# ukeSJTU/tiaozhanbei-unet

Hardware: AMD Instinct MI355X
Metric: training images/sec, AnomalyUNet 256x256 bs=32 per GPU (higher is better)
Workload: dtype bf16; 1 GPU; AnomalyUNet 3x256x256, bs=32/GPU, MSE+focal loss, Adam (BASELINE.json configs[2], synthetic randn images, bernoulli masks); global_batch=32, parallelism=dp1, accumulate=fp32, master_params=fp32, dist_world=1, reserved_cus=0, cu_budget=256

## Files before the change

tiaozhanbei_unet_amd/csrc/elementwise.hip:

```cpp
#include "common.h"

namespace {

inline int ew_blocks(long long items) { return (int)std::min<long long>(cdiv64(items, 256), 256 * 16); }

template <typename T>
__global__ __launch_bounds__(256) void nchw_to_nhwc_kernel(const float* __restrict__ src, T* __restrict__ dst,
                                                           int N, int C, int H, int W, int Cp) {
  constexpr int PIECE = ET<T>::PIECE;
  const long long hw = (long long)H * W;
  const long long total = (long long)N * hw;
  for (long long i = blockIdx.x * (long long)blockDim.x + threadIdx.x; i < total;
       i += (long long)gridDim.x * blockDim.x) {
    const long long n = i / hw, p = i - n * hw;
    const float* s = src + n * C * hw + p;
    T* o = dst + i * Cp;
    for (int c0 = 0; c0 < Cp; c0 += PIECE) {
      float v[PIECE];
#pragma unroll
      for (int j = 0; j < PIECE; ++j) v[j] = (c0 + j < C) ? s[(long long)(c0 + j) * hw] : 0.f;
      Vec<T>::store(o + c0, v);
    }
  }
}

template <typename T>
__global__ void nhwc_to_nchw_kernel(const T* __restrict__ src, float* __restrict__ dst, int N, int C, int H,
                                    int W, int Cp) {
  const long long hw = (long long)H * W;
  const long long total = (long long)N * C * hw;
  for (long long i = blockIdx.x * (long long)blockDim.x + threadIdx.x; i < total;
       i += (long long)gridDim.x * blockDim.x) {
    const long long p = i % hw;
    const long long t = i / hw;
    const int c = (int)(t % C);
    const long long n = t / C;
    dst[i] = ET<T>::to_f(src[(n * hw + p) * Cp + c]);
  }
}

template <typename T>
__global__ void pack_weight_kernel(const float* __restrict__ w, T* __restrict__ out, int Co, int Ci, int rows,
                                   int K, int mode, long long total, const float* __restrict__ scale) {
  for (long long i = blockIdx.x * (long long)blockDim.x + threadIdx.x; i < total;
       i += (long long)gridDim.x * blockDim.x) {
    float v = 0.f;
    if (mode == UNET_PACK_CONV_FWD) {
      const int ci = (int)(i % K);
      long long t = i / K;
      const int co = (int)(t % rows);
      const int tap = (int)(t / rows);
      if (co < Co && ci < Ci) v = w[((long long)co * Ci + ci) * 9 + tap] * (scale ? scale[co] : 1.f);
    } else if (mode == UNET_PACK_CONV_DGRAD) {
      const int co = (int)(i % K);
      long long t = i / K;
      const int ci = (int)(t % rows);
      const int tap = (int)(t / rows);
      if (co < Co && ci < Ci) v = w[((long long)co * Ci + ci) * 9 + (8 - tap)];
    } else if (mode == UNET_PACK_CONVT_FWD) {
      const int ci = (int)(i % K);
      long long t = i / K;
      const int co = (int)(t % rows);
      const int z = (int)(t / rows);
      if (co < Co && ci < Ci) v = w[((long long)ci * Co + co) * 4 + z];
    } else {
      const int co = (int)(i % K);
      long long t = i / K;
      const int z = (int)(t % 4);
      const int ci = (int)(t / 4);
      if (co < Co && ci < Ci) v = w[((long long)ci * Co + co) * 4 + z];
    }
    out[i] = ET<T>::from_f(v);
  }
}

template <typename T>
__global__ __launch_bounds__(256) void pack_weights_batched_kernel(const unet_pack_desc* __restrict__ descs) {
  __shared__ float tile[32 * 289];
  const unet_pack_desc d = descs[blockIdx.y];
  const int mode = d.mode;
  if (d.reserved > 0 && mode <= UNET_PACK_CONV_DGRAD) {
    const long long total = 9LL * d.rows * d.k;
    T* __restrict__ out = reinterpret_cast<T*>(d.out);
    for (long long i = blockIdx.x * 256LL + threadIdx.x; i < total; i += (long long)gridDim.x * 256)
      out[i] = ET<T>::from_f(unet_pack_seg_value(d.w, d.c_out, d.c_in, d.rows, d.k, mode, d.reserved, i, nullptr));
    return;
  }
  if constexpr (sizeof(T) == 2) {
    auto pair_ok = [](const unet_pack_desc& f, const unet_pack_desc& g) {
      return f.mode == UNET_PACK_CONV_FWD && g.mode == UNET_PACK_CONV_DGRAD && f.w == g.w && f.c_out == g.c_out &&
             f.c_in == g.c_in && f.rows == f.c_out && f.k == f.c_in && g.rows == g.c_in && g.k == g.c_out &&
             (f.c_out & 31) == 0 && (f.c_in & 31) == 0;
    };
    if (mode == UNET_PACK_CONV_DGRAD && blockIdx.y > 0 && pair_ok(descs[blockIdx.y - 1], d)) return;
    if (mode == UNET_PACK_CONV_FWD && blockIdx.y + 1 < gridDim.y && pair_ok(d, descs[blockIdx.y + 1])) {
      const unet_pack_desc g = descs[blockIdx.y + 1];
      const int Co = d.c_out, Ci = d.c_in;
      const int nB = Ci / 32, ntile = (Co / 32) * nB;
      const float* __restrict__ w = d.w;
      bf16_t* __restrict__ of = reinterpret_cast<bf16_t*>(d.out);
      bf16_t* __restrict__ og = reinterpret_cast<bf16_t*>(g.out);
      for (int t = blockIdx.x; t < ntile; t += gridDim.x) {
        const int a0 = (t / nB) * 32, b0 = (t % nB) * 32;
        __syncthreads();
        for (int i = threadIdx.x; i < 32 * 288; i += 256) {
          const int al = i / 288, r = i - al * 288;
          tile[al * 289 + r] = w[((size_t)(a0 + al) * Ci + b0) * 9 + r];
        }
        __syncthreads();
        for (int gi = threadIdx.x; gi < 2 * 32 * 9 * 4; gi += 256) {
          const int lay = gi / (32 * 9 * 4), rem = gi % (32 * 9 * 4);
          const int q = rem & 3, rest = rem >> 2;
          const int tap = rest % 9, outer = rest / 9;
          bf16x8 r8;
          if (lay == 0) {
#pragma unroll
            for (int e = 0; e < 8; ++e) r8[e] = (bf16_t)tile[outer * 289 + (q * 8 + e) * 9 + tap];
            *reinterpret_cast<bf16x8*>(of + ((size_t)tap * Co + a0 + outer) * Ci + b0 + q * 8) = r8;
          } else {
#pragma unroll
            for (int e = 0; e < 8; ++e) r8[e] = (bf16_t)tile[(q * 8 + e) * 289 + outer * 9 + tap];
            *reinterpret_cast<bf16x8*>(og + ((size_t)(8 - tap) * Ci + b0 + outer) * Co + a0 + q * 8) = r8;
          }
        }
      }
      return;
    }
  }
  const bool conv = mode <= UNET_PACK_CONV_DGRAD;
  const int taps = conv ? 9 : 4;
  const int As = conv ? d.c_out : d.c_in, Bs = conv ? d.c_in : d.c_out;
  const bool along_b = (mode == UNET_PACK_CONV_FWD || mode == UNET_PACK_CONVT_DGRAD);
  const int Ap = (mode == UNET_PACK_CONV_FWD || mode == UNET_PACK_CONVT_DGRAD) ? d.rows : d.k;
  const int Bp = (mode == UNET_PACK_CONV_FWD || mode == UNET_PACK_CONVT_DGRAD) ? d.k : d.rows;
  const int TA = along_b ? 8 : 64, TB = along_b ? 64 : 8;
  const int nA = (Ap + TA - 1) / TA, nB = (Bp + TB - 1) / TB;
  const float* __restrict__ w = d.w;
  T* __restrict__ out = reinterpret_cast<T*>(d.out);
  const int run = TB * taps;
  for (int t = blockIdx.x; t < nA * nB; t += gridDim.x) {
    const int a0 = (t / nB) * TA, b0 = (t % nB) * TB;
    __syncthreads();
    for (int i = threadIdx.x; i < TA * run; i += 256) {
      const int al = i / run, r = i - al * run;
      const int a = a0 + al, bb = b0 + r / taps;
      tile[i] = (a < As && bb < Bs) ? w[((size_t)a * Bs + b0) * taps + r] : 0.f;
    }
    __syncthreads();
    if ((((along_b ? Bp : Ap) & 7) == 0) && ((d.k & 7) == 0)) {
      for (int gi = threadIdx.x; gi < TA * TB * taps / 8; gi += 256) {
        const int inner0 = (gi & 7) * 8, rest = gi >> 3;
        const int tap = rest % taps, outer = rest / taps;
        const int al0 = along_b ? outer : inner0, bl0 = along_b ? inner0 : outer;
        const int a = a0 + al0, bb = b0 + bl0;
        if (a >= Ap || bb >= Bp) continue;
        float v[8];
#pragma unroll
        for (int e = 0; e < 8; ++e) v[e] = tile[(al0 + (along_b ? 0 : e)) * run + (bl0 + (along_b ? e : 0)) * taps + tap];
        size_t o;
        if (mode == UNET_PACK_CONV_FWD) o = ((size_t)tap * d.rows + a) * d.k + bb;
        else if (mode == UNET_PACK_CONV_DGRAD) o = ((size_t)(8 - tap) * d.rows + bb) * d.k + a;
        else if (mode == UNET_PACK_CONVT_FWD) o = ((size_t)tap * d.rows + bb) * d.k + a;
        else o = ((size_t)a * 4 + tap) * d.k + bb;
        if constexpr (sizeof(T) == 2) {
          bf16x8 r;
#pragma unroll
          for (int e = 0; e < 8; ++e) r[e] = (bf16_t)v[e];
          *reinterpret_cast<bf16x8*>(out + o) = r;
        } else {
          *reinterpret_cast<f32x4*>(out + o) = f32x4{v[0], v[1], v[2], v[3]};
          *reinterpret_cast<f32x4*>(out + o + 4) = f32x4{v[4], v[5], v[6], v[7]};
        }
      }
      continue;
    }
    for (int i = threadIdx.x; i < TA * TB * taps; i += 256) {
      const int inner = i & 63, rest = i >> 6;
      const int tap = rest % taps, outer = rest / taps;
      const int al = along_b ? outer : inner, bl = along_b ? inner : outer;
      const int a = a0 + al, bb = b0 + bl;
      if (a >= Ap || bb >= Bp) continue;
      const float v = tile[al * run + bl * taps + tap];
      size_t o;
      if (mode == UNET_PACK_CONV_FWD) o = ((size_t)tap * d.rows + a) * d.k + bb;
      else if (mode == UNET_PACK_CONV_DGRAD) o = ((size_t)(8 - tap) * d.rows + bb) * d.k + a;
      else if (mode == UNET_PACK_CONVT_FWD) o = ((size_t)tap * d.rows + bb) * d.k + a;
      else o = ((size_t)a * 4 + tap) * d.k + bb;
      out[o] = ET<T>::from_f(v);
    }
  }
}

template <typename T>
__global__ void maxpool2_fwd_kernel(const T* __restrict__ x, T* __restrict__ y, int N, int H, int W, int C) {
  constexpr int PIECE = ET<T>::PIECE;
  const int OH = H / 2, OW = W / 2, G = C / PIECE;
  const long long total = (long long)N * OH * OW * G;
  for (long long i = blockIdx.x * (long long)blockDim.x + threadIdx.x; i < total;
       i += (long long)gridDim.x * blockDim.x) {
    const int g = (int)(i % G);
    long long t = i / G;
    const int ox = (int)(t % OW);  t /= OW;
    const int oy = (int)(t % OH);
    const long long n = t / OH;
    const T* p = x + ((n * H + 2 * oy) * W + 2 * ox) * (long long)C + g * PIECE;
    float a[PIECE], b[PIECE], c[PIECE], d[PIECE];
    Vec<T>::load(p, a);
    Vec<T>::load(p + C, b);
    Vec<T>::load(p + (long long)W * C, c);
    Vec<T>::load(p + (long long)W * C + C, d);
#pragma unroll
    for (int j = 0; j < PIECE; ++j) a[j] = fmaxf(fmaxf(a[j], b[j]), fmaxf(c[j], d[j]));
    Vec<T>::store(y + i * PIECE, a);
  }
}

template <typename T>
__global__ void maxpool2_bwd_kernel(const T* __restrict__ x, const T* __restrict__ dy, T* __restrict__ dx,
                                    int N, int H, int W, int C, int accumulate) {
  constexpr int PIECE = ET<T>::PIECE;
  const int OH = H / 2, OW = W / 2, G = C / PIECE;
  const int WH = (H + 1) / 2, WW = (W + 1) / 2;
  const long long total = (long long)N * WH * WW * G;
  for (long long i = blockIdx.x * (long long)blockDim.x + threadIdx.x; i < total;
       i += (long long)gridDim.x * blockDim.x) {
    const int g = (int)(i % G);
    long long t = i / G;
    const int ox = (int)(t % WW);  t /= WW;
    const int oy = (int)(t % WH);
    const long long n = t / WH;
    const long long base = ((n * H + 2 * oy) * W + 2 * ox) * (long long)C + g * PIECE;
    float z[PIECE];
#pragma unroll
    for (int j = 0; j < PIECE; ++j) z[j] = 0.f;
    if (oy < OH && ox < OW) {
      float a[PIECE], b[PIECE], c[PIECE], d[PIECE], gr[PIECE];
      Vec<T>::load(x + base, a);
      Vec<T>::load(x + base + C, b);
      Vec<T>::load(x + base + (long long)W * C, c);
      Vec<T>::load(x + base + (long long)W * C + C, d);
      Vec<T>::load(dy + (((n * OH + oy) * OW + ox) * (long long)C + g * PIECE), gr);
      float ga[PIECE], gb[PIECE], gc[PIECE], gd[PIECE];
// ... 347 lines not shown
    using T = decltype(tag);
    return ew_launch("nchw_to_nhwc_kernel", nchw_to_nhwc_kernel<T>, (long long)n * h * w, UNET_K_PACK, stream, src, (T*)dst,
                     n, c, h, w, c_pad);
  });
}

extern "C" int32_t unet_nhwc_to_nchw(const void* src, float* dst, int32_t n, int32_t c, int32_t h, int32_t w,
                                     int32_t c_pad, int32_t dtype, void* stream) {
  UNET_REQUIRE(src && dst, UNET_ERR_BAD_ARG, "unet_nhwc_to_nchw: null pointer");
  UNET_REQUIRE(n > 0 && c > 0 && h > 0 && w > 0 && c_pad >= c, UNET_ERR_BAD_ARG, "unet_nhwc_to_nchw: bad dims");
  return with_dtype("unet_nhwc_to_nchw", dtype, [&](auto tag) {
    using T = decltype(tag);
    return ew_launch("nhwc_to_nchw_kernel", nhwc_to_nchw_kernel<T>, (long long)n * h * w * c, UNET_K_PACK, stream,
                     (const T*)src, dst, n, c, h, w, c_pad);
  });
}

static int32_t launch_pack_weight(const char* who, int dtype, const float* w, void* out, int c_out, int c_in, int rows, int k,
                                  int mode, int taps, const float* scale, void* stream) {
  const long long total = (long long)taps * rows * k;
  return with_dtype(who, dtype, [&](auto tag) {
    using T = decltype(tag);
    return ew_launch("pack_weight_kernel", pack_weight_kernel<T>, total, UNET_K_PACK, stream, w, (T*)out, c_out, c_in, rows,
                     k, mode, total, scale);
  });
}

extern "C" int32_t unet_pack_weight(const float* w, void* out, int32_t c_out, int32_t c_in, int32_t rows,
                                    int32_t k, int32_t mode, int32_t dtype, void* stream) {
  UNET_REQUIRE(w && out, UNET_ERR_BAD_ARG, "unet_pack_weight: null pointer");
  UNET_REQUIRE(c_out > 0 && c_in > 0 && rows > 0 && k > 0 && mode >= 0 && mode <= 3, UNET_ERR_BAD_ARG,
               "unet_pack_weight: bad dims/mode");
  const int gemm_rows = (mode == UNET_PACK_CONV_FWD || mode == UNET_PACK_CONVT_FWD) ? c_out : c_in;
  const int gemm_k = (mode == UNET_PACK_CONV_FWD || mode == UNET_PACK_CONVT_FWD) ? c_in : c_out;
  UNET_REQUIRE(rows >= gemm_rows && k >= gemm_k, UNET_ERR_BAD_ARG, "unet_pack_weight: padded dims too small");
  const int taps = (mode <= UNET_PACK_CONV_DGRAD) ? 9 : 4;
  return launch_pack_weight("unet_pack_weight", dtype, w, out, c_out, c_in, rows, k, mode, taps, nullptr, stream);
}

extern "C" int32_t unet_pack_conv_weight_folded(const float* w, const float* scale, void* out, int32_t c_out, int32_t c_in,
                                                int32_t rows, int32_t k, int32_t dtype, void* stream) {
  UNET_REQUIRE(w && scale && out, UNET_ERR_BAD_ARG, "unet_pack_conv_weight_folded: null pointer");
  UNET_REQUIRE(c_out > 0 && c_in > 0 && rows >= c_out && k >= c_in, UNET_ERR_BAD_ARG, "unet_pack_conv_weight_folded: bad dims");
  return launch_pack_weight("unet_pack_conv_weight_folded", dtype, w, out, c_out, c_in, rows, k, UNET_PACK_CONV_FWD, 9, scale,
                            stream);
}

extern "C" int32_t unet_pack_weights_batched(const unet_pack_desc* descs, int32_t n, int32_t dtype, void* stream) {
  UNET_REQUIRE(descs && n > 0 && n <= 65535, UNET_ERR_BAD_ARG, "unet_pack_weights_batched: bad argument");
  hipStream_t s = (hipStream_t)stream;
  return with_dtype("unet_pack_weights_batched", dtype, [&](auto tag) {
    using T = decltype(tag);
    ProfScope prof(UNET_K_PACK, 0.0, s);
    hipLaunchKernelGGL(pack_weights_batched_kernel<T>, dim3(224, n), dim3(256), 0, s, descs);
    return unet_check_launch("pack_weights_batched_kernel");
  });
}

extern "C" int32_t unet_maxpool2_fwd(int32_t dtype, const void* x, int32_t n, int32_t h, int32_t w, int32_t c,
                                     void* y, void* stream) {
  UNET_REQUIRE(x && y, UNET_ERR_BAD_ARG, "unet_maxpool2_fwd: null pointer");
  UNET_REQUIRE(n > 0 && h >= 2 && w >= 2 && c > 0 && c % 8 == 0, UNET_ERR_UNSUPPORTED, "unet_maxpool2_fwd: dims");
  return with_dtype("unet_maxpool2_fwd", dtype, [&](auto tag) {
    using T = decltype(tag);
    const long long total = (long long)n * (h / 2) * (w / 2) * c / ET<T>::PIECE;
    return ew_launch("maxpool2_fwd_kernel", maxpool2_fwd_kernel<T>, total, UNET_K_POOL, stream, (const T*)x, (T*)y, n, h, w, c);
  });
}

extern "C" int32_t unet_maxpool2_bwd(int32_t dtype, const void* x, const void* dy, int32_t n, int32_t h,
                                     int32_t w, int32_t c, void* dx, int32_t accumulate, void* stream) {
  UNET_REQUIRE(x && dy && dx, UNET_ERR_BAD_ARG, "unet_maxpool2_bwd: null pointer");
  UNET_REQUIRE(n > 0 && h >= 2 && w >= 2 && c > 0 && c % 8 == 0, UNET_ERR_UNSUPPORTED, "unet_maxpool2_bwd: dims");
  return with_dtype("unet_maxpool2_bwd", dtype, [&](auto tag) {
    using T = decltype(tag);
    const long long total = (long long)n * ((h + 1) / 2) * ((w + 1) / 2) * c / ET<T>::PIECE;
    return ew_launch("maxpool2_bwd_kernel", maxpool2_bwd_kernel<T>, total, UNET_K_POOL, stream, (const T*)x, (const T*)dy,
                     (T*)dx, n, h, w, c, accumulate);
  });
}

extern "C" int32_t unet_bn_relu_pool_supported(int32_t dtype, int32_t c) {
  if (!dtype_known(dtype)) return 0;
  const int piece = dtype == UNET_BF16 ? ET<bf16_t>::PIECE : ET<float>::PIECE;
  return (c > 0 && c % piece == 0 && 256 % (c / piece) == 0) ? 1 : 0;
}

template <typename T> using PoolIdx32 = std::conditional_t<sizeof(T) == 2, int, long long>;

extern "C" int32_t unet_bn_relu_pool_fwd(int32_t dtype, const void* y, int32_t n, int32_t h, int32_t w, int32_t c,
                                         const float* scale, const float* shift, void* a, void* pooled, void* stream) {
  UNET_REQUIRE(y && scale && shift && a && pooled, UNET_ERR_BAD_ARG, "unet_bn_relu_pool_fwd: null pointer");
  hipStream_t s = (hipStream_t)stream;
  return with_dtype("unet_bn_relu_pool_fwd", dtype, [&](auto tag) -> int32_t {
    using T = decltype(tag);
    UNET_REQUIRE(n > 0 && h >= 2 && w >= 2 && unet_bn_relu_pool_supported(dtype, c), UNET_ERR_UNSUPPORTED,
                 "unet_bn_relu_pool_fwd: c=%d h=%d w=%d", c, h, w);
    ProfScope prof(UNET_K_BN, 0.0, s, "bn_relu_pool_fwd_kernel");
    const long long total = (long long)n * ((h + 1) / 2) * ((w + 1) / 2) * (c / ET<T>::PIECE);
    const dim3 grid(ew_blocks(total));
    if ((long long)n * h * w * c < 0x7FFFFFFFLL)
      hipLaunchKernelGGL((bn_relu_pool_fwd_kernel<T, PoolIdx32<T>>), grid, dim3(256), 0, s, (const T*)y, scale, shift, (T*)a,
                         (T*)pooled, n, h, w, c);
    else
      hipLaunchKernelGGL((bn_relu_pool_fwd_kernel<T, long long>), grid, dim3(256), 0, s, (const T*)y, scale, shift, (T*)a,
                         (T*)pooled, n, h, w, c);
    return unet_check_launch("bn_relu_pool_fwd_kernel");
// ... 274 lines not shown
```

tiaozhanbei_unet_amd/csrc/first.hip:

```cpp
#include <stdlib.h>

#include <algorithm>

#include "conv_common.h"

namespace {

constexpr unsigned OOB = 0xFFFFFFF0u;
constexpr int FIRST_CO = 64;

struct SegPos { int seg, y, n; };
__device__ __forceinline__ SegPos seg_step(SegPos p, int dseg, int dy, int dn, int segs_row, int H) {
  p.seg += dseg;
  int c = p.seg >= segs_row;
  p.seg -= c ? segs_row : 0;
  p.y += dy + c;
  c = p.y >= H;
  p.y -= c ? H : 0;
  p.n += dn + c;
  return p;
}
struct SegWalk { SegPos first; int dseg, dy, dn; };
__device__ __forceinline__ SegWalk seg_walk(long long u0, long long stride, int segs_row, int H) {
  SegWalk w;
  const long long r0 = u0 / segs_row, rs = stride / segs_row;
  w.first = SegPos{(int)(u0 - r0 * segs_row), (int)(r0 % H), (int)std::min<long long>(r0 / H, 1 << 30)};
  w.dseg = (int)(stride - rs * segs_row);
  w.dy = (int)(rs % H);
  w.dn = (int)std::min<long long>(rs / H, 1 << 28);
  return w;
}

struct FirstParams {
  const float* x;
  const float* w;
  char* y;
  float* part;
  int N, CI, H, W;
  const char* y_raw;
  const float* coefs;
};

__global__ __launch_bounds__(256, 3) void first_fwd_kernel(const FirstParams P) {
  __shared__ float red[4][2][FIRST_CO];
  const int tid = threadIdx.x, lane = tid & 63, wave = tid >> 6;
  const int l15 = lane & 15, kb = lane >> 4;
  const int K = 9 * P.CI;
  const int HW = P.H * P.W;

  bf16x8 wa[4];
#pragma unroll
  for (int ct = 0; ct < 4; ++ct)
#pragma unroll
    for (int e = 0; e < 8; ++e) {
      const int k = kb * 8 + e;
      float v = 0.f;
      if (k < K) {
// ... 247 lines not shown
  for (int i = 0; i < WU; ++i) issue_or_skip(seg_step(cur, i, 0, 0, segs_row, P.H), i, xc[i]);
  while (cur.n < P.N) {
    const SegPos nxt = seg_step(cur, wk.dseg, wk.dy, wk.dn, segs_row, P.H);
#pragma unroll
    for (int i = 0; i < WU; ++i) issue_or_skip(seg_step(nxt, i, 0, 0, segs_row, P.H), (buf ^ 1) * WU + i, xn[i]);
    asm volatile("s_waitcnt vmcnt(%0)" ::"n"(NV * WU) : "memory");
#pragma unroll
    for (int i = 0; i < WU; ++i) {
      bf16x8 fb;
#pragma unroll
      for (int e = 0; e < 8; ++e) fb[e] = (bf16_t)xc[i][e];
      const char* sb = wbuf + (buf * WU + i) * SEGB;
#pragma unroll
      for (int wr = 0; wr < 2; ++wr) {
        bf16x8 fa = tr_frag2(sb, aoff[wr], aoff[wr] + 4 * 128);
        if constexpr (BNB) {
          const bf16x8 fy = tr_frag2(sb + 2048, aoff[wr], aoff[wr] + 4 * 128);
#pragma unroll
          for (int e = 0; e < 8; ++e)
            fa[e] = (bf16_t)fmaf(cA[wr], (float)fa[e], fmaf(cB[wr], (float)fy[e], cK[wr]));
        }
        acc[wr] = __builtin_amdgcn_mfma_f32_32x32x16_bf16(fa, fb, acc[wr], 0, 0, 0);
      }
    }
#pragma unroll
    for (int i = 0; i < WU; ++i)
#pragma unroll
      for (int e = 0; e < 8; ++e) xc[i][e] = xn[i][e];
    buf ^= 1;
    cur = nxt;
  }
  asm volatile("s_waitcnt vmcnt(0)" ::: "memory");

  __syncthreads();
  float* red = reinterpret_cast<float*>(smem);
#pragma unroll
  for (int wr = 0; wr < 2; ++wr)
#pragma unroll
    for (int r = 0; r < 16; ++r) {
      const int co = wr * 32 + (r & 3) + 8 * (r >> 2) + 4 * hh;
      red[(wave * FIRST_CO + co) * 32 + l31] = acc[wr][r];
    }
  __syncthreads();
  for (int i = tid; i < FIRST_CO * 32; i += 256) {
    const float t = ((red[i] + red[FIRST_CO * 32 + i]) + red[2 * FIRST_CO * 32 + i]) + red[3 * FIRST_CO * 32 + i];
    P.part[(size_t)blockIdx.x * (FIRST_CO * 32) + i] = t;
  }
}

__global__ __launch_bounds__(256) void first_wgrad_reduce_kernel(const float* __restrict__ part, int nparts, int CI,
                                                                 float* __restrict__ dw) {
  __shared__ float red[8][32];
  const int co = blockIdx.x, k = threadIdx.x & 31, pl = threadIdx.x >> 5;
  float s0 = 0.f, s1 = 0.f;
  int b = pl;
  for (; b + 8 < nparts; b += 16) {
    s0 += part[(size_t)b * (FIRST_CO * 32) + co * 32 + k];
    s1 += part[(size_t)(b + 8) * (FIRST_CO * 32) + co * 32 + k];
  }
  if (b < nparts) s0 += part[(size_t)b * (FIRST_CO * 32) + co * 32 + k];
  red[pl][k] = s0 + s1;
  __syncthreads();
  if (threadIdx.x < 9 * CI) {
    const int kk = threadIdx.x, tap = kk / CI, ci = kk - tap * CI;
    float t = red[0][kk];
#pragma unroll
    for (int i = 1; i < 8; ++i) t += red[i][kk];
    dw[(co * CI + ci) * 9 + tap] = t;
  }
}

int first_blocks(long long units, int per_iter, int per_cu) {
  long long b = (units + 4 * per_iter - 1) / (4 * per_iter);
  return (int)std::min<long long>(b, 256 * per_cu);
}

}

extern "C" int32_t unet_conv3x3_first_supported(int32_t c_in, int32_t c_out, int32_t h, int32_t w) {
  return (c_in >= 1 && 9 * c_in <= 32 && c_out == FIRST_CO && h > 0 && w > 0 && w % 16 == 0) ? 1 : 0;
}

extern "C" int32_t unet_conv3x3_first_stats(int32_t n, int32_t h, int32_t w, const float* x, int32_t c_in,
                                            const float* weight, void* y, float* partial, int32_t* n_parts,
                                            void* stream) {
  UNET_REQUIRE(x && weight && y, UNET_ERR_BAD_ARG, "unet_conv3x3_first_stats: null pointer");
  UNET_REQUIRE(n > 0 && unet_conv3x3_first_supported(c_in, FIRST_CO, h, w), UNET_ERR_UNSUPPORTED,
               "unet_conv3x3_first_stats: n=%d c_in=%d h=%d w=%d (needs 9*c_in <= 32, w %% 16 == 0)", n, c_in, h, w);
  UNET_REQUIRE((long long)c_in * h * w * 4 < 0x7FFFFFFFLL, UNET_ERR_UNSUPPORTED, "unet_conv3x3_first_stats: image too large");
  const long long units = (long long)n * h * (w / 16);
  const int blocks = first_blocks(units, 2, 3);
  FirstParams P{x, weight, (char*)y, partial, n, c_in, h, w, nullptr, nullptr};
  hipStream_t s = (hipStream_t)stream;
  ProfScope prof(UNET_K_CONV_FWD, 2.0 * n * h * w * (double)FIRST_CO * c_in * 9, s);
  hipLaunchKernelGGL(first_fwd_kernel, dim3(blocks), dim3(256), 0, s, P);
  if (n_parts) *n_parts = partial ? blocks : 0;
  return unet_check_launch("first_fwd_kernel");
}

extern "C" size_t unet_conv3x3_first_wgrad_workspace(int32_t n, int32_t h, int32_t w) {
  const long long units = (long long)n * h * (w / 16 > 0 ? w / 16 : 1);
  return (size_t)first_blocks(units, 2, 4) * FIRST_CO * 32 * sizeof(float);
}

static int32_t first_wgrad_impl(int32_t n, int32_t h, int32_t w, const float* x, int32_t c_in, const void* dy, const void* y_raw,
                                const float* coefs, float* dw, void* workspace, size_t workspace_bytes, void* stream,
                                const char* what) {
  UNET_REQUIRE(x && dy && dw && workspace, UNET_ERR_BAD_ARG, "%s: null pointer", what);
  UNET_REQUIRE(n > 0 && unet_conv3x3_first_supported(c_in, FIRST_CO, h, w), UNET_ERR_UNSUPPORTED,
               "%s: n=%d c_in=%d h=%d w=%d", what, n, c_in, h, w);
  UNET_REQUIRE((long long)c_in * h * w * 4 < 0x7FFFFFFFLL, UNET_ERR_UNSUPPORTED, "%s: image too large", what);
  UNET_REQUIRE(workspace_bytes >= unet_conv3x3_first_wgrad_workspace(n, h, w), UNET_ERR_WORKSPACE, "%s: workspace too small", what);
  const long long units = (long long)n * h * (w / 16);
  const int blocks = first_blocks(units, 2, 4);
// ... 26 lines not shown
```

tiaozhanbei_unet_amd/csrc/wgrad.hip:

```cpp
#include <stdlib.h>

#include <algorithm>

#include "common.h"

namespace {

struct WView { const char* p; int C, H, W, oy, ox; };

#ifdef PDMA_STAMPS
void* g_wgrad_debug = nullptr;
#endif
struct WgradParams {
  void* debug;
  WView rt;
  WView ct[2];
  int N, H, W;
  int Crow, Ccol;
  float* partial;
  int split, tilesPerSplit, tilesX, tilesY, nR, nC;
  int xcd_chunk;
};

__device__ inline bool wgrad_block_coords(const WgradParams& P, int& sp, int& rtile, int& ctile) {
// ... 629 lines not shown
#pragma unroll
  for (int tap = 0; tap < 9; ++tap) {
    float* o = P.partial + ((size_t)(sp * 9 + tap) * P.Crow) * P.Ccol;
#pragma unroll
    for (int cb = 0; cb < 2; ++cb)
#pragma unroll
      for (int nb = 0; nb < 2; ++nb) {
        const int row = rch + wr * 32 + cb * 16 + i16;
        const int col = ctile * 64 + wc * 32 + nb * 16 + g * 4;
        *reinterpret_cast<f32x4*>(o + (size_t)row * P.Ccol + col) = acc[tap][cb][nb];
      }
  }
  asm volatile("s_waitcnt vmcnt(0)" ::: "memory");
#ifdef PDMA_STAMPS
  if (P.debug && lane == 0 && blockIdx.x < 256) {
    unsigned long long* o = (unsigned long long*)P.debug + ((size_t)blockIdx.x * 8 + wave) * 8;
    for (int i = 0; i < 4; ++i) o[i] = wg_st[i];
    o[4] = (unsigned long long)(t_end - t_begin);
    o[5] = ((__builtin_amdgcn_s_memtime() - wg_t0) << 20) / (__builtin_amdgcn_s_memrealtime() - wg_r0 + 1);
    o[6] = __builtin_amdgcn_s_memtime() - wg_e0;
    o[7] = __builtin_amdgcn_s_memtime() - wg_t0;
  }
#endif
}

template <int TAPS>
__global__ __launch_bounds__(256) void wgrad_reduce_wide_kernel(const float* __restrict__ partial,
                                                                float* __restrict__ out, int split, int Crow,
                                                                int Ccol, int rows_out, int cols_out) {
  __shared__ float red[4][64];
  const int cl = threadIdx.x & 63, ks = threadIdx.x >> 6;
  int b = blockIdx.x;
  const int tap = b % TAPS;  b /= TAPS;
  const int nchunk = (cols_out + 63) / 64;
  const int c = (b % nchunk) * 64 + cl, r = b / nchunk;
  const size_t plane = (size_t)Crow * Ccol, slab = (size_t)TAPS * plane;
  float s = 0.f;
  if (c < cols_out) {
    const float* p = partial + (size_t)tap * plane + (size_t)r * Ccol + c;
    int k = ks;
    for (; k + 12 < split; k += 16) {
      const float a0 = p[(size_t)k * slab], a1 = p[(size_t)(k + 4) * slab], a2 = p[(size_t)(k + 8) * slab],
                  a3 = p[(size_t)(k + 12) * slab];
      s += a0; s += a1; s += a2; s += a3;
    }
    for (; k < split; k += 4) s += p[(size_t)k * slab];
  }
  red[ks][cl] = s;
  __syncthreads();
  if (ks == 0 && c < cols_out)
    out[((size_t)r * cols_out + c) * TAPS + tap] = (red[0][cl] + red[1][cl]) + (red[2][cl] + red[3][cl]);
}

struct Plan { int tilesX, tilesY, nR, nC, split, tilesPerSplit; size_t bytes; };

template <int TAPS>
Plan make_plan(int n, int h, int w, int crow, int ccol) {
  Plan p;
  constexpr int TH = (TAPS == 9) ? 8 : 4;
  p.tilesX = cdiv(w, 16);
  p.tilesY = cdiv(h, TH);
  p.nR = crow / 64;
  p.nC = ccol / 64;
  const long long ntiles = (long long)n * p.tilesY * p.tilesX;
  long long want = 2LL * unet_cu_budget() / ((long long)p.nR * p.nC);
  if (want < 1) want = 1;
  if (want > ntiles) want = ntiles;
  p.tilesPerSplit = (int)cdiv64(ntiles, want);
  p.split = (int)cdiv64(ntiles, p.tilesPerSplit);
  p.bytes = (size_t)p.split * TAPS * crow * ccol * sizeof(float);
  return p;
}

inline Plan make_plan16(int n, int h, int w, int crow, int ccol) {
  Plan p;
  const bool paired = w <= 16;
  p.tilesX = paired ? 1 : cdiv(w, 32);
  p.tilesY = cdiv(h, 4);
  p.nR = crow / 128;
  p.nC = ccol / 64;
  const long long ntiles = (long long)(paired ? (n + 1) / 2 : n) * p.tilesY * p.tilesX;
  long long want = (long long)unet_cu_budget() / ((long long)p.nR * p.nC);
  if (want < 1) want = 1;
  if (want > ntiles) want = ntiles;
  p.tilesPerSplit = (int)cdiv64(ntiles, want);
  p.split = (int)cdiv64(ntiles, p.tilesPerSplit);
  p.bytes = (size_t)p.split * 9 * crow * ccol * sizeof(float);
  return p;
}

template <bool PAIRED>
void launch16(const WgradParams& P, long long blocks, hipStream_t s) {
  using C = W16<PAIRED>;
  auto kern = wgrad16_kernel<PAIRED>;
  unet_set_max_lds(reinterpret_cast<const void*>(kern), C::LDS);
  hipLaunchKernelGGL(kern, dim3((unsigned)blocks), dim3(512), C::LDS, s, P);
}

template <typename T, int TAPS>
int32_t run(WgradParams& P, const Plan& pl, float* out, int rows_out, int cols_out, int kclass, hipStream_t s) {
  P.tilesX = pl.tilesX; P.tilesY = pl.tilesY; P.nR = pl.nR; P.nC = pl.nC;
  P.split = pl.split; P.tilesPerSplit = pl.tilesPerSplit;
  long long blocks = (long long)pl.split * pl.nR * pl.nC;
  P.xcd_chunk = 0;
  if (blocks >= 16) {
    P.xcd_chunk = (int)cdiv64(blocks, 8);
    blocks = 8LL * P.xcd_chunk;
  }
  const double flops = 2.0 * P.N * P.H * P.W * (double)P.Crow * P.Ccol * TAPS;
  int split_used = pl.split;
  {
    const double alg_bytes = (double)P.N * P.H * P.W * ((double)P.Crow + P.Ccol * (TAPS == 9 ? 1.0 : 4.0)) * sizeof(T) +
                             4.0 * TAPS * rows_out * cols_out;
    constexpr bool DMA = sizeof(T) == 2 && TAPS == 9;
    const bool v16 = DMA && P.Crow % 128 == 0;
    ProfScope prof(kclass, flops, s,
                   v16 ? "wgrad16_kernel (+ reduce)" : (DMA ? "wgrad_dma_kernel (+ reduce)" : "wgrad_kernel (+ reduce)"), alg_bytes);
    if constexpr (DMA) {
      if (v16) {
        const Plan p16 = make_plan16(P.N, P.H, P.W, P.Crow, P.Ccol);
        P.tilesX = p16.tilesX; P.tilesY = p16.tilesY; P.nR = p16.nR; P.nC = p16.nC;
        P.split = p16.split; P.tilesPerSplit = p16.tilesPerSplit;
        split_used = p16.split;
        long long b16 = (long long)p16.split * p16.nR * p16.nC;
        P.xcd_chunk = 0;
        if (b16 >= 16) { P.xcd_chunk = (int)cdiv64(b16, 8); b16 = 8LL * P.xcd_chunk; }
        if (P.W <= 16) launch16<true>(P, b16, s);
        else launch16<false>(P, b16, s);
      } else {
        unet_set_max_lds(reinterpret_cast<const void*>(wgrad_dma_kernel), WDma::LDS);
        hipLaunchKernelGGL(wgrad_dma_kernel, dim3((unsigned)blocks), dim3(256), WDma::LDS, s, P);
      }
    } else {
      using C = WCfg<T, TAPS>;
      auto kern = wgrad_kernel<T, TAPS>;
      unet_set_max_lds(reinterpret_cast<const void*>(kern), C::LDS);
      hipLaunchKernelGGL(kern, dim3((unsigned)blocks), dim3(256), C::LDS, s, P);
    }
    int32_t rc = unet_check_launch("wgrad_kernel");
    if (rc) return rc;
    if (split_used >= 16) {
      const long long rb = (long long)rows_out * ((cols_out + 63) / 64) * TAPS;
      hipLaunchKernelGGL(wgrad_reduce_wide_kernel<TAPS>, dim3((unsigned)rb), dim3(256), 0, s, (const float*)P.partial,
                         out, split_used, P.Crow, P.Ccol, rows_out, cols_out);
    } else {
      const long long total = (long long)rows_out * cols_out;
      const int rb = (int)std::min<long long>(cdiv64(total, 256), 4096);
      hipLaunchKernelGGL(wgrad_reduce_kernel<TAPS>, dim3(rb), dim3(256), 0, s, (const float*)P.partial, out, split_used,
                         P.Crow, P.Ccol, rows_out, cols_out);
    }
  }
  return unet_check_launch("wgrad_reduce_kernel");
}

inline int pad64(int c) { return (c + 63) / 64 * 64; }

}

extern "C" size_t unet_conv3x3_wgrad_workspace(int32_t n, int32_t h, int32_t w, int32_t c_in, int32_t c_out) {
  size_t bytes = make_plan<9>(n, h, w, pad64(c_out), pad64(c_in)).bytes;
  if (pad64(c_out) % 128 == 0)
    bytes = std::max(bytes, make_plan16(n, h, w, pad64(c_out), pad64(c_in)).bytes);
  return bytes;
}

extern "C" int32_t unet_conv3x3_wgrad(int32_t dtype, int32_t n, int32_t h, int32_t w, const unet_view src[2],
                                      const void* dy, int32_t c_out, float* dw, int32_t c_in_param,
                                      void* workspace, size_t workspace_bytes, void* stream) {
  UNET_REQUIRE(src && src[0].ptr && dy && dw && workspace, UNET_ERR_BAD_ARG, "unet_conv3x3_wgrad: null pointer");
  UNET_REQUIRE(n > 0 && h > 0 && w > 0, UNET_ERR_BAD_ARG, "unet_conv3x3_wgrad: bad dims");
  const int ctot = src[0].c + (src[1].ptr ? src[1].c : 0);
  UNET_REQUIRE(c_out % 64 == 0, UNET_ERR_UNSUPPORTED, "unet_conv3x3_wgrad: c_out %d not a multiple of 64", c_out);
  UNET_REQUIRE(ctot % 64 == 0 && (!src[1].ptr || src[0].c % 64 == 0), UNET_ERR_UNSUPPORTED,
               "unet_conv3x3_wgrad: input channels %d(+%d) must be multiples of 64", src[0].c,
               src[1].ptr ? src[1].c : 0);
  UNET_REQUIRE(c_in_param <= ctot, UNET_ERR_BAD_ARG, "unet_conv3x3_wgrad: c_in_param %d > %d", c_in_param, ctot);
  const Plan pl = make_plan<9>(n, h, w, c_out, ctot);
  const size_t need = unet_conv3x3_wgrad_workspace(n, h, w, ctot, c_out);
  UNET_REQUIRE(workspace_bytes >= need, UNET_ERR_WORKSPACE, "unet_conv3x3_wgrad: workspace %zu < %zu", workspace_bytes, need);
  WgradParams P{};
#ifdef PDMA_STAMPS
  P.debug = g_wgrad_debug;
#endif
  P.rt = WView{(const char*)dy, c_out, h, w, 0, 0};
  P.ct[0] = WView{(const char*)src[0].ptr, src[0].c, src[0].h, src[0].w, src[0].off_y, src[0].off_x};
  P.ct[1] = src[1].ptr ? WView{(const char*)src[1].ptr, src[1].c, src[1].h, src[1].w, src[1].off_y, src[1].off_x}
                       : WView{nullptr, 0, 0, 0, 0, 0};
  P.N = n; P.H = h; P.W = w;
  P.Crow = c_out; P.Ccol = ctot;
  P.partial = (float*)workspace;
  hipStream_t s = (hipStream_t)stream;
  return with_dtype("unet_conv3x3_wgrad", dtype, [&](auto tag) {
    return run<decltype(tag), 9>(P, pl, dw, c_out, c_in_param, UNET_K_CONV_WGRAD, s);
  });
// ... 273 lines not shown
```

Before: 1860 images/sec.

## Rework weight packing into a flat tile scheduler and vectorize wgrad reductions

Replaces the 2D-grid weight packing kernel with a single persistent grid that prefix-scans per-descriptor tile counts and walks a flat tile list. The paired fwd/dgrad path moves to 64x64 tiles staged in LDS as bf16 using vectorized global loads. It also adds a vectorized float4 wgrad split-reduce kernel for small split counts, with an LDS transpose so stores are coalesced, and a software-pipelined split_sum helper for the first-layer reduction. These target launch imbalance and scalar memory traffic in per-step weight packing and reductions. The cost is more complex indexing and extra LDS use.

```diff
diff --git a/tiaozhanbei_unet_amd/csrc/elementwise.hip b/tiaozhanbei_unet_amd/csrc/elementwise.hip
--- a/tiaozhanbei_unet_amd/csrc/elementwise.hip
+++ b/tiaozhanbei_unet_amd/csrc/elementwise.hip
@@ -74,120 +74,196 @@
   }
 }
 
+constexpr int PACK_SEG_CHUNK = 256 * 16;
+constexpr int PACK_PAIR_RS = 64 * 9 + 2;
+constexpr int PACK_LDS = 64 * PACK_PAIR_RS * 2;
+
+__device__ inline bool pack_pair_ok(const unet_pack_desc& f, const unet_pack_desc& g) {
+  return f.mode == UNET_PACK_CONV_FWD && g.mode == UNET_PACK_CONV_DGRAD && f.w == g.w && f.c_out == g.c_out &&
+         f.c_in == g.c_in && f.rows == f.c_out && f.k == f.c_in && g.rows == g.c_in && g.k == g.c_out &&
+         f.reserved <= 0 && g.reserved <= 0 && (f.c_out & 63) == 0 && (f.c_in & 63) == 0 &&
+         (((uintptr_t)f.w | (uintptr_t)f.out | (uintptr_t)g.out) & 15) == 0;
+}
+
 template <typename T>
-__global__ __launch_bounds__(256) void pack_weights_batched_kernel(const unet_pack_desc* __restrict__ descs) {
-  __shared__ float tile[32 * 289];
-  const unet_pack_desc d = descs[blockIdx.y];
+__device__ inline int pack_tile_count(const unet_pack_desc* __restrict__ descs, int n, int i, bool* paired) {
+  const unet_pack_desc d = descs[i];
+  *paired = false;
+  if (d.reserved > 0 && d.mode <= UNET_PACK_CONV_DGRAD) return (int)((9LL * d.rows * d.k + PACK_SEG_CHUNK - 1) / PACK_SEG_CHUNK);
+  if constexpr (sizeof(T) == 2) {
+    if (d.mode == UNET_PACK_CONV_DGRAD && i > 0 && pack_pair_ok(descs[i - 1], d)) return 0;
+    if (d.mode == UNET_PACK_CONV_FWD && i + 1 < n && pack_pair_ok(d, descs[i + 1])) {
+      *paired = true;
+      return (d.c_out / 64) * (d.c_in / 64);
+    }
+  }
+  const bool along_b = (d.mode == UNET_PACK_CONV_FWD || d.mode == UNET_PACK_CONVT_DGRAD);
+  const int Ap = along_b ? d.rows : d.k, Bp = along_b ? d.k : d.rows;
+  const int TA = along_b ? 8 : 64, TB = along_b ? 64 : 8;
+  return ((Ap + TA - 1) / TA) * ((Bp + TB - 1) / TB);
+}
+
+__device__ inline void pack_pair_tile(const unet_pack_desc& d, const unet_pack_desc& g, int t, bf16_t* __restrict__ lds) {
+  constexpr int RS = PACK_PAIR_RS;
+  const int Co = d.c_out, Ci = d.c_in, nB = Ci / 64;
+  const int a0 = (t / nB) * 64, b0 = (t % nB) * 64;
+  typedef __attribute__((address_space(1))) const f32x4 g_f32x4;
+  typedef __attribute__((address_space(1))) bf16x8 g_bf16x8;
+  const float* w = d.w + ((size_t)a0 * Ci + b0) * 9;
+  bf16_t* of = reinterpret_cast<bf16_t*>(d.out);
+  bf16_t* og = reinterpret_cast<bf16_t*>(g.out);
+#pragma unroll 1
+  for (int j0 = 0; j0 < 36; j0 += 12) {
+    f32x4 v[12];
+#pragma unroll
+    for (int j = 0; j < 12; ++j) {
+      const int i = threadIdx.x + 256 * (j0 + j), row = i / 144, r4 = i - row * 144;
+      v[j] = *(g_f32x4*)(w + (size_t)row * Ci * 9 + r4 * 4);
+    }
+#pragma unroll
+    for (int j = 0; j < 12; ++j) {
+      const int i = threadIdx.x + 256 * (j0 + j), row = i / 144, r4 = i - row * 144;
+      bf16x4 h;
+#pragma unroll
+      for (int e = 0; e < 4; ++e) h[e] = (bf16_t)v[j][e];
+      const u32x2 u = __builtin_bit_cast(u32x2, h);
+      uint32_t* q = reinterpret_cast<uint32_t*>(lds + row * RS + r4 * 4);
+      q[0] = u[0];
+      q[1] = u[1];
+    }
+  }
+  __syncthreads();
+#pragma unroll 2
+  for (int j = 0; j < 18; ++j) {
+    const int gi = threadIdx.x + 256 * j;
+    const int q = gi & 7, co = (gi >> 3) & 63, tap = gi >> 9;
+    bf16x8 r8;
+#pragma unroll
+    for (int e = 0; e < 8; ++e) r8[e] = lds[co * RS + (q * 8 + e) * 9 + tap];
+    *(g_bf16x8*)(of + ((size_t)tap * Co + a0 + co) * Ci + b0 + q * 8) = r8;
+  }
+#pragma unroll 2
+  for (int j = 0; j < 18; ++j) {
+    const int gi = threadIdx.x + 256 * j;
+    const int q = (gi & 3) | ((gi >> 3) & 4), ci = ((gi >> 2) & 7) | ((gi >> 3) & 56), tap = gi >> 9;
+    bf16x8 r8;
+#pragma unroll
+    for (int e = 0; e < 8; ++e) r8[e] = lds[(q * 8 + e) * RS + ci * 9 + tap];
+    *(g_bf16x8*)(og + ((size_t)(8 - tap) * Ci + b0 + ci) * Co + a0 + q * 8) = r8;
+  }
+}
+
+template <typename T>
+__device__ inline void pack_generic_tile(const unet_pack_desc& d, int t, float* __restrict__ tile) {
   const int mode = d.mode;
-  if (d.reserved > 0 && mode <= UNET_PACK_CONV_DGRAD) {
-    const long long total = 9LL * d.rows * d.k;
-    T* __restrict__ out = reinterpret_cast<T*>(d.out);
-    for (long long i = blockIdx.x * 256LL + threadIdx.x; i < total; i += (long long)gridDim.x * 256)
-      out[i] = ET<T>::from_f(unet_pack_seg_value(d.w, d.c_out, d.c_in, d.rows, d.k, mode, d.reserved, i, nullptr));
-    return;
-  }
-  if constexpr (sizeof(T) == 2) {
-    auto pair_ok = [](const unet_pack_desc& f, const unet_pack_desc& g) {
-      return f.mode == UNET_PACK_CONV_FWD && g.mode == UNET_PACK_CONV_DGRAD && f.w == g.w && f.c_out == g.c_out &&
-             f.c_in == g.c_in && f.rows == f.c_out && f.k == f.c_in && g.rows == g.c_in && g.k == g.c_out &&
-             (f.c_out & 31) == 0 && (f.c_in & 31) == 0;
-    };
-    if (mode == UNET_PACK_CONV_DGRAD && blockIdx.y > 0 && pair_ok(descs[blockIdx.y - 1], d)) return;
-    if (mode == UNET_PACK_CONV_FWD && blockIdx.y + 1 < gridDim.y && pair_ok(d, descs[blockIdx.y + 1])) {
-      const unet_pack_desc g = descs[blockIdx.y + 1];
-      const int Co = d.c_out, Ci = d.c_in;
-      const int nB = Ci / 32, ntile = (Co / 32) * nB;
-      const float* __restrict__ w = d.w;
-      bf16_t* __restrict__ of = reinterpret_cast<bf16_t*>(d.out);
-      bf16_t* __restrict__ og = reinterpret_cast<bf16_t*>(g.out);
-      for (int t = blockIdx.x; t < ntile; t += gridDim.x) {
-        const int a0 = (t / nB) * 32, b0 = (t % nB) * 32;
-        __syncthreads();
-        for (int i = threadIdx.x; i < 32 * 288; i += 256) {
-          const int al = i / 288, r = i - al * 288;
-          tile[al * 289 + r] = w[((size_t)(a0 + al) * Ci + b0) * 9 + r];
-        }
-        __syncthreads();
-        for (int gi = threadIdx.x; gi < 2 * 32 * 9 * 4; gi += 256) {
-          const int lay = gi / (32 * 9 * 4), rem = gi % (32 * 9 * 4);
-          const int q = rem & 3, rest = rem >> 2;
-          const int tap = rest % 9, outer = rest / 9;
-          bf16x8 r8;
-          if (lay == 0) {
-#pragma unroll
-            for (int e = 0; e < 8; ++e) r8[e] = (bf16_t)tile[outer * 289 + (q * 8 + e) * 9 + tap];
-            *reinterpret_cast<bf16x8*>(of + ((size_t)tap * Co + a0 + outer) * Ci + b0 + q * 8) = r8;
-          } else {
-#pragma unroll
-            for (int e = 0; e < 8; ++e) r8[e] = (bf16_t)tile[(q * 8 + e) * 289 + outer * 9 + tap];
-            *reinterpret_cast<bf16x8*>(og + ((size_t)(8 - tap) * Ci + b0 + outer) * Co + a0 + q * 8) = r8;
-          }
-        }
-      }
-      return;
-    }
-  }
   const bool conv = mode <= UNET_PACK_CONV_DGRAD;
   const int taps = conv ? 9 : 4;
   const int As = conv ? d.c_out : d.c_in, Bs = conv ? d.c_in : d.c_out;
   const bool along_b = (mode == UNET_PACK_CONV_FWD || mode == UNET_PACK_CONVT_DGRAD);
-  const int Ap = (mode == UNET_PACK_CONV_FWD || mode == UNET_PACK_CONVT_DGRAD) ? d.rows : d.k;
-  const int Bp = (mode == UNET_PACK_CONV_FWD || mode == UNET_PACK_CONVT_DGRAD) ? d.k : d.rows;
+  const int Ap = along_b ? d.rows : d.k;
+  const int Bp = along_b ? d.k : d.rows;
   const int TA = along_b ? 8 : 64, TB = along_b ? 64 : 8;
-  const int nA = (Ap + TA - 1) / TA, nB = (Bp + TB - 1) / TB;
+  const int nB = (Bp + TB - 1) / TB;
   const float* __restrict__ w = d.w;
   T* __restrict__ out = reinterpret_cast<T*>(d.out);
   const int run = TB * taps;
-  for (int t = blockIdx.x; t < nA * nB; t += gridDim.x) {
-    const int a0 = (t / nB) * TA, b0 = (t % nB) * TB;
-    __syncthreads();
-    for (int i = threadIdx.x; i < TA * run; i += 256) {
-      const int al = i / run, r = i - al * run;
-      const int a = a0 + al, bb = b0 + r / taps;
-      tile[i] = (a < As && bb < Bs) ? w[((size_t)a * Bs + b0) * taps + r] : 0.f;
-    }
-    __syncthreads();
-    if ((((along_b ? Bp : Ap) & 7) == 0) && ((d.k & 7) == 0)) {
-      for (int gi = threadIdx.x; gi < TA * TB * taps / 8; gi += 256) {
-        const int inner0 = (gi & 7) * 8, rest = gi >> 3;
-        const int tap = rest % taps, outer = rest / taps;
-        const int al0 = along_b ? outer : inner0, bl0 = along_b ? inner0 : outer;
-        const int a = a0 + al0, bb = b0 + bl0;
-        if (a >= Ap || bb >= Bp) continue;
-        float v[8];
-#pragma unroll
-        for (int e = 0; e < 8; ++e) v[e] = tile[(al0 + (along_b ? 0 : e)) * run + (bl0 + (along_b ? e : 0)) * taps + tap];
-        size_t o;
-        if (mode == UNET_PACK_CONV_FWD) o = ((size_t)tap * d.rows + a) * d.k + bb;
-        else if (mode == UNET_PACK_CONV_DGRAD) o = ((size_t)(8 - tap) * d.rows + bb) * d.k + a;
-        else if (mode == UNET_PACK_CONVT_FWD) o = ((size_t)tap * d.rows + bb) * d.k + a;
-        else o = ((size_t)a * 4 + tap) * d.k + bb;
-        if constexpr (sizeof(T) == 2) {
-          bf16x8 r;
-#pragma unroll
-          for (int e = 0; e < 8; ++e) r[e] = (bf16_t)v[e];
-          *reinterpret_cast<bf16x8*>(out + o) = r;
-        } else {
-          *reinterpret_cast<f32x4*>(out + o) = f32x4{v[0], v[1], v[2], v[3]};
-          *reinterpret_cast<f32x4*>(out + o + 4) = f32x4{v[4], v[5], v[6], v[7]};
-        }
-      }
-      continue;
-    }
-    for (int i = threadIdx.x; i < TA * TB * taps; i += 256) {
-      const int inner = i & 63, rest = i >> 6;
+  const int a0 = (t / nB) * TA, b0 = (t % nB) * TB;
+  for (int i = threadIdx.x; i < TA * run; i += 256) {
+    const int al = i / run, r = i - al * run;
+    const int a = a0 + al, bb = b0 + r / taps;
+    tile[i] = (a < As && bb < Bs) ? w[((size_t)a * Bs + b0) * taps + r] : 0.f;
+  }
+  __syncthreads();
+  if ((((along_b ? Bp : Ap) & 7) == 0) && ((d.k & 7) == 0) && ((uintptr_t)d.out & 15) == 0) {
+    for (int gi = threadIdx.x; gi < TA * TB * taps / 8; gi += 256) {
+      const int inner0 = (gi & 7) * 8, rest = gi >> 3;
       const int tap = rest % taps, outer = rest / taps;
-      const int al = along_b ? outer : inner, bl = along_b ? inner : outer;
-      const int a = a0 + al, bb = b0 + bl;
+      const int al0 = along_b ? outer : inner0, bl0 = along_b ? inner0 : outer;
+      const int a = a0 + al0, bb = b0 + bl0;
       if (a >= Ap || bb >= Bp) continue;
-      const float v = tile[al * run + bl * taps + tap];
+      float v[8];
+#pragma unroll
+      for (int e = 0; e < 8; ++e) v[e] = tile[(al0 + (along_b ? 0 : e)) * run + (bl0 + (along_b ? e : 0)) * taps + tap];
       size_t o;
       if (mode == UNET_PACK_CONV_FWD) o = ((size_t)tap * d.rows + a) * d.k + bb;
       else if (mode == UNET_PACK_CONV_DGRAD) o = ((size_t)(8 - tap) * d.rows + bb) * d.k + a;
       else if (mode == UNET_PACK_CONVT_FWD) o = ((size_t)tap * d.rows + bb) * d.k + a;
       else o = ((size_t)a * 4 + tap) * d.k + bb;
-      out[o] = ET<T>::from_f(v);
-    }
+      if constexpr (sizeof(T) == 2) {
+        bf16x8 r;
+#pragma unroll
+        for (int e = 0; e < 8; ++e) r[e] = (bf16_t)v[e];
+        *reinterpret_cast<bf16x8*>(out + o) = r;
+      } else {
+        *reinterpret_cast<f32x4*>(out + o) = f32x4{v[0], v[1], v[2], v[3]};
+        *reinterpret_cast<f32x4*>(out + o + 4) = f32x4{v[4], v[5], v[6], v[7]};
+      }
+    }
+    return;
+  }
+  for (int i = threadIdx.x; i < TA * TB * taps; i += 256) {
+    const int inner = i & 63, rest = i >> 6;
+    const int tap = rest % taps, outer = rest / taps;
+    const int al = along_b ? outer : inner, bl = along_b ? inner : outer;
+    const int a = a0 + al, bb = b0 + bl;
+    if (a >= Ap || bb >= Bp) continue;
+    const float v = tile[al * run + bl * taps + tap];
+    size_t o;
+    if (mode == UNET_PACK_CONV_FWD) o = ((size_t)tap * d.rows + a) * d.k + bb;
+    else if (mode == UNET_PACK_CONV_DGRAD) o = ((size_t)(8 - tap) * d.rows + bb) * d.k + a;
+    else if (mode == UNET_PACK_CONVT_FWD) o = ((size_t)tap * d.rows + bb) * d.k + a;
+    else o = ((size_t)a * 4 + tap) * d.k + bb;
+    out[o] = ET<T>::from_f(v);
+  }
+}
+
+template <typename T>
+__global__ __launch_bounds__(256) void pack_weights_batched_kernel(const unet_pack_desc* __restrict__ descs, int n) {
+  extern __shared__ __attribute__((aligned(16))) char pack_smem[];
+  __shared__ int scan[2][256];
+  __shared__ int first[257];
+  long long done = 0;
+  for (int base = 0; base < n; base += 256) {
+    const int i = base + threadIdx.x;
+    bool paired = false;
+    const int cnt = i < n ? pack_tile_count<T>(descs, n, i, &paired) : 0;
+    __syncthreads();
+    scan[0][threadIdx.x] = cnt;
+    __syncthreads();
+    int pp = 0;
+    for (int off = 1; off < 256; off <<= 1) {
+      const int v = scan[pp][threadIdx.x] + (threadIdx.x >= off ? scan[pp][threadIdx.x - off] : 0);
+      scan[pp ^ 1][threadIdx.x] = v;
+      pp ^= 1;
+      __syncthreads();
+    }
+    first[threadIdx.x + 1] = scan[pp][threadIdx.x];
+    if (threadIdx.x == 0) first[0] = 0;
+    __syncthreads();
+    const int chunk_tiles = first[256];
+    long long t = blockIdx.x - done % gridDim.x;
+    if (t < 0) t += gridDim.x;
+    for (; t < chunk_tiles; t += gridDim.x) {
+      int lo = 0, hi = 255;
+      while (lo < hi) {
+        const int mid = (lo + hi + 1) >> 1;
+        if (first[mid] <= (int)t) lo = mid; else hi = mid - 1;
+      }
+      const unet_pack_desc d = descs[base + lo];
+      const int lt = (int)t - first[lo];
+      __syncthreads();
+      if (d.reserved > 0 && d.mode <= UNET_PACK_CONV_DGRAD) {
+        const long long total = 9LL * d.rows * d.k, e0 = (long long)lt * PACK_SEG_CHUNK;
+        T* __restrict__ out = reinterpret_cast<T*>(d.out);
+        for (long long e = e0 + threadIdx.x; e < total && e < e0 + PACK_SEG_CHUNK; e += 256)
+          out[e] = ET<T>::from_f(unet_pack_seg_value(d.w, d.c_out, d.c_in, d.rows, d.k, d.mode, d.reserved, e, nullptr));
+      } else if (sizeof(T) == 2 && d.mode == UNET_PACK_CONV_FWD && base + lo + 1 < n && pack_pair_ok(d, descs[base + lo + 1])) {
+        pack_pair_tile(d, descs[base + lo + 1], lt, reinterpret_cast<bf16_t*>(pack_smem));
+      } else {
+        pack_generic_tile<T>(d, lt, reinterpret_cast<float*>(pack_smem));
+      }
+    }
+    done += chunk_tiles;
   }
 }
 
@@ -641,7 +717,11 @@
   return with_dtype("unet_pack_weights_batched", dtype, [&](auto tag) {
     using T = decltype(tag);
     ProfScope prof(UNET_K_PACK, 0.0, s);
-    hipLaunchKernelGGL(pack_weights_batched_kernel<T>, dim3(224, n), dim3(256), 0, s, descs);
+    constexpr bool pairs = sizeof(T) == 2;
+    constexpr int lds = pairs ? PACK_LDS : 32 * 289 * (int)sizeof(float);
+    auto kern = pack_weights_batched_kernel<T>;
+    unet_set_max_lds(reinterpret_cast<const void*>(kern), lds);
+    hipLaunchKernelGGL(kern, dim3(pairs ? 512 : 1024), dim3(256), lds, s, descs, (int)n);
     return unet_check_launch("pack_weights_batched_kernel");
   });
 }
diff --git a/tiaozhanbei_unet_amd/csrc/first.hip b/tiaozhanbei_unet_amd/csrc/first.hip
--- a/tiaozhanbei_unet_amd/csrc/first.hip
+++ b/tiaozhanbei_unet_amd/csrc/first.hip
@@ -3,6 +3,7 @@
 #include <algorithm>
 
 #include "conv_common.h"
+#include "split_sum.h"
 
 namespace {
 
@@ -356,14 +357,9 @@
                                                                  float* __restrict__ dw) {
   __shared__ float red[8][32];
   const int co = blockIdx.x, k = threadIdx.x & 31, pl = threadIdx.x >> 5;
-  float s0 = 0.f, s1 = 0.f;
-  int b = pl;
-  for (; b + 8 < nparts; b += 16) {
-    s0 += part[(size_t)b * (FIRST_CO * 32) + co * 32 + k];
-    s1 += part[(size_t)(b + 8) * (FIRST_CO * 32) + co * 32 + k];
-  }
-  if (b < nparts) s0 += part[(size_t)b * (FIRST_CO * 32) + co * 32 + k];
-  red[pl][k] = s0 + s1;
+  float s[2] = {0.f, 0.f};
+  split_sum<2, 16>(part + co * 32 + k, (size_t)FIRST_CO * 32, pl, 8, 16, nparts, s);
+  red[pl][k] = s[0] + s[1];
   __syncthreads();
   if (threadIdx.x < 9 * CI) {
     const int kk = threadIdx.x, tap = kk / CI, ci = kk - tap * CI;
diff --git a/tiaozhanbei_unet_amd/csrc/split_sum.h b/tiaozhanbei_unet_amd/csrc/split_sum.h
--- /dev/null
+++ b/tiaozhanbei_unet_amd/csrc/split_sum.h
@@ -0,0 +1,53 @@
+#pragma once
+#include "common.h"
+
+constexpr int SPLIT_SUM_W = 4;
+
+template <typename V>
+__device__ inline V split_sum_load(const float* p) { return *reinterpret_cast<const V*>(p); }
+
+template <int NCH, int D, typename V>
+__device__ inline void split_sum(const float* __restrict__ p, size_t stride, int first, int cstep, int istep, int n,
+                                 V (&acc)[NCH]) {
+  V a[D][NCH];
+  if (n == SPLIT_SUM_W * D * istep && first + (NCH - 1) * cstep < istep) {
+#pragma unroll
+    for (int w = 0; w < SPLIT_SUM_W; ++w)
+#pragma unroll
+      for (int i = 0; i < D; ++i)
+#pragma unroll
+        for (int j = 0; j < NCH; ++j) {
+          if (w == 0) a[i][j] = split_sum_load<V>(p + (size_t)(first + j * cstep + i * istep) * stride);
+        }
+#pragma unroll
+    for (int w = 0; w < SPLIT_SUM_W; ++w)
+#pragma unroll
+      for (int i = 0; i < D; ++i)
+#pragma unroll
+        for (int j = 0; j < NCH; ++j) {
+          acc[j] += a[i][j];
+          if (w + 1 < SPLIT_SUM_W)
+            a[i][j] = split_sum_load<V>(p + (size_t)(first + j * cstep + ((w + 1) * D + i) * istep) * stride);
+          __builtin_amdgcn_sched_barrier(0);
+        }
+    return;
+  }
+#pragma unroll
+  for (int i = 0; i < D; ++i)
+#pragma unroll
+    for (int j = 0; j < NCH; ++j) {
+      const int kk = first + j * cstep + i * istep;
+      a[i][j] = split_sum_load<V>(p + (size_t)(kk < n ? kk : 0) * stride);
+    }
+  for (int k = first; k < n; k += D * istep) {
+#pragma unroll
+    for (int i = 0; i < D; ++i)
+#pragma unroll
+      for (int j = 0; j < NCH; ++j) {
+        const int kk = k + j * cstep + i * istep, nx = kk + D * istep;
+        if (kk < n) acc[j] += a[i][j];
+        a[i][j] = split_sum_load<V>(p + (size_t)(nx < n ? nx : 0) * stride);
+        __builtin_amdgcn_sched_barrier(0);
+      }
+  }
+}
diff --git a/tiaozhanbei_unet_amd/csrc/wgrad.hip b/tiaozhanbei_unet_amd/csrc/wgrad.hip
--- a/tiaozhanbei_unet_amd/csrc/wgrad.hip
+++ b/tiaozhanbei_unet_amd/csrc/wgrad.hip
@@ -705,6 +705,55 @@
     out[((size_t)r * cols_out + c) * TAPS + tap] = (red[0][cl] + red[1][cl]) + (red[2][cl] + red[3][cl]);
 }
 
+template <int TAPS>
+__global__ __launch_bounds__(256) void wgrad_reduce4_kernel(const float* __restrict__ partial, float* __restrict__ out,
+                                                            int split, int Crow, int Ccol, int rows_out, int cols_out) {
+  __shared__ f32x4 turn[4][64 * TAPS];
+  const int lane = threadIdx.x & 63, wave = threadIdx.x >> 6;
+  const int nq = cols_out / 4;
+  const long long quads = (long long)rows_out * nq;
+  const long long wave0 = (long long)blockIdx.x * 256 + wave * 64;
+  const long long i = wave0 + lane < quads ? wave0 + lane : quads - 1;
+  const int c = (int)(i % nq) * 4, r = (int)(i / nq);
+  const size_t plane = (size_t)Crow * Ccol, slab = (size_t)TAPS * plane;
+  const float* p = partial + (size_t)r * Ccol + c;
+  f32x4 s[TAPS];
+#pragma unroll
+  for (int t = 0; t < TAPS; ++t) s[t] = f32x4{0.f, 0.f, 0.f, 0.f};
+  int k = 0;
+  for (; k + 1 < split; k += 2) {
+    f32x4 a[2][TAPS];
+#pragma unroll
+    for (int u = 0; u < 2; ++u)
+#pragma unroll
+      for (int t = 0; t < TAPS; ++t) a[u][t] = *reinterpret_cast<const f32x4*>(p + (size_t)(k + u) * slab + (size_t)t * plane);
+#pragma unroll
+    for (int u = 0; u < 2; ++u)
+#pragma unroll
+      for (int t = 0; t < TAPS; ++t) s[t] += a[u][t];
+  }
+  if (k < split) {
+    f32x4 a[TAPS];
+#pragma unroll
+    for (int t = 0; t < TAPS; ++t) a[t] = *reinterpret_cast<const f32x4*>(p + (size_t)k * slab + (size_t)t * plane);
+#pragma unroll
+    for (int t = 0; t < TAPS; ++t) s[t] += a[t];
+  }
+#pragma unroll
+  for (int j = 0; j < TAPS; ++j) {
+    f32x4 v;
+#pragma unroll
+    for (int e = 0; e < 4; ++e) v[e] = s[(4 * j + e) % TAPS][(4 * j + e) / TAPS];
+    turn[wave][lane * TAPS + j] = v;
+  }
+  __syncthreads();
+#pragma unroll
+  for (int j = 0; j < TAPS; ++j) {
+    const int idx = j * 64 + lane;
+    if (wave0 + idx / TAPS < quads) *reinterpret_cast<f32x4*>(out + ((size_t)wave0 * TAPS + idx) * 4) = turn[wave][idx];
+  }
+}
+
 struct Plan { int tilesX, tilesY, nR, nC, split, tilesPerSplit; size_t bytes; };
 
 template <int TAPS>
@@ -792,7 +841,12 @@
     }
     int32_t rc = unet_check_launch("wgrad_kernel");
     if (rc) return rc;
-    if (split_used >= 16) {
+    const bool vec = (((uintptr_t)P.partial | (uintptr_t)out) & 15) == 0 && cols_out % 4 == 0 && rows_out > 0 && cols_out > 0;
+    if (vec && split_used < 16) {
+      const long long rb = cdiv64((long long)rows_out * (cols_out / 4), 256);
+      hipLaunchKernelGGL(wgrad_reduce4_kernel<TAPS>, dim3((unsigned)rb), dim3(256), 0, s, (const float*)P.partial, out,
+                         split_used, P.Crow, P.Ccol, rows_out, cols_out);
+    } else if (split_used >= 16) {
       const long long rb = (long long)rows_out * ((cols_out + 63) / 64) * TAPS;
       hipLaunchKernelGGL(wgrad_reduce_wide_kernel<TAPS>, dim3((unsigned)rb), dim3(256), 0, s, (const float*)P.partial,
                          out, split_used, P.Crow, P.Ccol, rows_out, cols_out);
```

Result: slower. 1841 images/sec (-1.0%).
